# zyang1580/PDA

Hardware: AMD Instinct MI355X
Metric: users/sec full-catalogue top-K@50 (eval) (higher is better)
Workload: dtype f32; 1 GPU; C3: synthetic 1000000 users x 200000 items, d=128, PDA condition ((elu+1)*pop^0.22) head, masked top-K@50; ranks_seen=1

## Files before the change

### include/pda_hip_experimental.h

```cpp
#ifndef PDA_HIP_EXPERIMENTAL_H
#define PDA_HIP_EXPERIMENTAL_H

#include "pda_hip.h"

#ifdef __cplusplus
extern "C" {
#endif

int pda_score_topk_huge_splits(int n_users_blk, int n_items_local, int d);

int pda_topk_kth_value(const uint64_t* keys, int n_splits, int n_users_blk, int K, int pos, float* out, void* stream);
int pda_topk_remap_items(uint64_t* keys, size_t n_keys, const int32_t* gid, int n_gid, void* stream);
int pda_topk_seed_bounds(const uint64_t* keys, int n_splits, int n_users_blk, int K, int m, float* bounds, void* stream);
int pda_topk_seed_counts(const uint64_t* keys, int n_splits, int n_users_blk, int K, const float* bounds, int n_thr, int32_t* counts,
                         void* stream);
int pda_topk_seed_pick(const float* bounds, const int32_t* counts, int n_thr, int n_users_blk, int K, float* seed, void* stream);
int pda_topk_seed_refine(const uint64_t* keys, int n_splits, int n_users_blk, int K, float* lo, float* hi, float* mid, int32_t* counts,
                         int mode, void* stream);
int pda_score_topk4_phase_f32(const float* U, const float* I_shard, const void* prep, const float* pop_shard, const int32_t* users,
                              int n_users_blk, int item_offset, int n_items_local, int d, const int64_t* hist_indptr,
                              const int32_t* hist_indices, int hist_row_mode, int K, int head, int early_stop, int n_splits,
                              int phase, int warm_tiles, const float* seed, uint64_t* out_keys, void* workspace, void* stream);
int pda_score_topk4_phase_bf16(const uint16_t* U, const uint16_t* I_shard, const void* prep, const float* pop_shard,
                               const int32_t* users, int n_users_blk, int item_offset, int n_items_local, int d,
                               const int64_t* hist_indptr, const int32_t* hist_indices, int hist_row_mode, int K, int head,
                               int early_stop, int n_splits, int phase, int warm_tiles, const float* seed, uint64_t* out_keys,
                               void* workspace, void* stream);
int pda_score_topk4_phase_image_offsets(int n_users_blk, int n_items_local, int d, int n_splits, size_t* offs);
int pda_score_topk4_phase_user_image(const void* U, int bf16, const int32_t* users, int n_users_blk, int d, void* ufrag, float* unorm,
                                     void* stream);
int pda_score_topk4_phase_mask_table(const void* prep, int n_items_local, int d, int item_offset, const int64_t* hist_indptr,
                                     const int32_t* hist_indices, int n_rows, uint32_t* table, void* stream);
int pda_score_topk4_phase_masked_f32(const float* U, const float* I_shard, const void* prep, const float* pop_shard, const int32_t* users,
                                     int n_users_blk, int item_offset, int n_items_local, int d, const int64_t* hist_indptr,
                                     const int32_t* hist_indices, int hist_row_mode, int K, int head, int early_stop, int n_splits,
                                     const uint32_t* mask_table, int mask_table_rows, uint64_t* out_keys, void* workspace, void* stream);
int pda_score_topk4_phase_masked_bf16(const uint16_t* U, const uint16_t* I_shard, const void* prep, const float* pop_shard, const int32_t* users,
                                      int n_users_blk, int item_offset, int n_items_local, int d, const int64_t* hist_indptr,
                                      const int32_t* hist_indices, int hist_row_mode, int K, int head, int early_stop, int n_splits,
                                      const uint32_t* mask_table, int mask_table_rows, uint64_t* out_keys, void* workspace, void* stream);
int pda_score_topk4_phase_mask_rows(const void* prep, const int32_t* users, int n_users_blk, int item_offset, int n_items_local, int d,
                                    const int64_t* hist_indptr, const int32_t* hist_indices, int hist_row_mode, int warm_tiles, uint32_t* out,
                                    void* stream);
int pda_score_topk4_phase_mask_offsets(int n_users_blk, int n_items_local, int d, int n_splits, size_t* offs);

size_t pda_triplet_plan_bytes(int B);
size_t pda_triplet_plan_large_workspace_bytes(int B);
int pda_triplet_plan_large(const int32_t* users, const int32_t* pos, const int32_t* neg, int B, void* plan, void* workspace, void* stream);
size_t pda_bpr_step_plan_scratch_bytes(int B, int d);
int pda_triplet_plan(const int32_t* users, const int32_t* pos, const int32_t* neg, int B, int n_batches, void* plans, void* stream);
int pda_bpr_step_plan_f32(float* U, float* I, const int32_t* users, const int32_t* pos, const int32_t* neg, const float* pos_pop,
                          const float* neg_pop, int B, int d, float regs, float reg_div, float lr, const void* plan, float* scratch,
                          int exact, float* loss_acc, void* stream);
int pda_bpr_step_plan_bf16(uint16_t* U_bf16, uint16_t* I_bf16, float* U_master, float* I_master, const int32_t* users,
                           const int32_t* pos, const int32_t* neg, const float* pos_pop, const float* neg_pop, int B, int d,
                           float regs, float reg_div, float lr, const void* plan, float* scratch, float* loss_acc, void* stream);

int pda_sort_triplets_by_pos(int32_t* users, int32_t* pos, int32_t* neg, float* pos_pop, float* neg_pop, int B,
                             void* stream);

int pda_group_triplets_by_pos(int32_t* users, int32_t* pos, int32_t* neg, float* pos_pop, float* neg_pop, int B,
                              void* stream);

int pda_adam_mark_rows(const int32_t* users, const int32_t* pos, const int32_t* neg, int B, uint32_t* touched_u, uint32_t* touched_i, void* stream);
int pda_adam_dense_sweep3_f32(float* var_a, float* m_a, float* v_a, float* g_a, size_t rows_a, uint32_t* touched_a, float* var_b, float* m_b, float* v_b,
                              float* g_b, size_t rows_b, uint32_t* touched_b, int d, float lr_t, float beta1, float beta2, float eps, void* stream);

int pda_adam_rows_f32(float* var, float* m, float* v, float* g, const int32_t* rows, int n_rows, int d, float lr_t,
                      float beta1, float beta2, float eps, void* stream);

int pda_adam_lazy_f32(int phase, float* U, float* mU, float* vU, float* gU, int32_t* lastU, float* I, float* mI, float* vI,
                      float* gI, int32_t* lastI, const int32_t* users, const int32_t* pos, const int32_t* neg, int B, int d, int t,
                      const float* lr_tab, float beta1, float beta2, float eps, void* stream);
int pda_adam_lazy_sync_f32(float* var, float* m, float* v, int32_t* last, size_t n_rows, int d, int t, const float* lr_tab,
                           float beta1, float beta2, float eps, void* stream);
int pda_adam_lazy_dev_f32(int phase, float* U, float* mU, float* vU, float* gU, int32_t* lastU, float* I, float* mI, float* vI,
                          float* gI, int32_t* lastI, const int32_t* users, const int32_t* pos, const int32_t* neg, int B, int d,
// ... 41 lines not shown
```

### pda_amd/csrc/pda_score_topk_v4.hip

```cpp
#include "pda_v4_shared.h"
#include <cstdlib>
#include <type_traits>

using namespace pda_topk;

namespace {

constexpr int kCap4 = 57;
constexpr int kRing4 = 128;
constexpr int kWarmTiles = 4;
constexpr int kMainWaves = 8;
#ifndef PDA_W4_ABL
#define PDA_W4_ABL 0
#endif
#ifndef PDA_V4_ABL
#define PDA_V4_ABL 0
#endif
#ifdef PDA_V4_PROF
__device__ unsigned long long pda_prof4[24];
#define PROF_T0(v) const long long v = __builtin_readcyclecounter()
#define PROF_T1(v, slot) prof[slot] += (unsigned long long)(__builtin_readcyclecounter() - v)
#define PROF_INC(slot, x) prof[slot] += (unsigned long long)(x)
#define PROF_FLUSH(first, last) do { if (lane == 0) for (int pq = (first); pq <= (last); ++pq) atomicAdd(&pda_prof4[pq], prof[pq]); } while (0)
#else
// ... 17 lines not shown
    const float* sufA;
    const float* sufB;
    const int* pos_of;
    unsigned* stats;
    uint64_t* lists_ws;
    int32_t* regroup_ws;
    float* pred_ws;
    const int32_t* row_perm;
    const uint32_t* hmask_ws;
    const uint32_t* bloom;
    const int* prep_hdr;
    const float* seed;
    int n_users_blk, item_offset, n_items_local, hist_row_mode, K, n_splits, n_tiles;
    int warm_tiles;
    int warm_sorted;
    uint64_t* handover;
    const unsigned char* rows5;
    const float* meta5;
    const unsigned char* ufrag;
    const float* unorm;
    int prep_hdr_pop;
    int warm_final;
    int warm_shared;
    float* seed_out;
    const int* n_users_dev;
    int lists_empty;
    const float* tailA;
    const float* tailB;
    unsigned char* ufrag_out;
    float* unorm_out;
    float* kth_ws;
    const uint32_t* hmask_tab;
    int hmask_tab_rows;
};


template <int D, bool BF>
__global__ void __launch_bounds__(256) prep4_kernel(const void* __restrict__ I, const float* __restrict__ pop, const int* __restrict__ order,
                                                    int n, int n_pad, unsigned char* __restrict__ rows, int* __restrict__ pos_of,
                                                    int* __restrict__ hdr, unsigned char* __restrict__ rows5, int* __restrict__ meta5, u32x4* __restrict__ pinfo,
                                                    int f16img) {
    constexpr int TPR = D / 8, RB = row_bytes(D);
    const int pos = blockIdx.x * (256 / TPR) + threadIdx.x / TPR, e = threadIdx.x % TPR;
    if (pos >= n_pad) return;
    unsigned char* rp = rows + (size_t)pos * RB;
    float ss = 0.f, popv = 1.0f, rs = 0.f;
    int src = -1;
    if (pos < n) {
        src = pos;
        if (order) {
            src = order[pos];
            if (src < 0 || src >= n) { if (e == 0) atomicOr(hdr, 1); src = 0; }
            else if (e == 0 && atomicExch(&pos_of[src], pos) != -1) atomicOr(hdr, 1);
        } else if (e == 0) {
            pos_of[pos] = pos;
        }
        if (pop) popv = pop[src];
        const f32x4 a = pda_load4<BF>(I, (size_t)src * D + 8 * e);
        const f32x4 b = pda_load4<BF>(I, (size_t)src * D + 8 * e + 4);
        u32x4 hq, lq;
        split8(a, b, hq, lq);
        *reinterpret_cast<u32x4*>(rp + 16 * e) = hq;
#pragma unroll
        for (int k = 0; k < 4; ++k) ss += a[k] * a[k] + b[k] * b[k];
        {
            const float pv = pop ? ((popv == popv) ? popv : 0.f) : 1.0f;
// ... 571 lines not shown
        }
        if (g.kth_ws != nullptr) continue;
        if (g.handover != nullptr) {
            if (rb < g.n_users_blk && lane < CAP) g.handover[((size_t)split * g.n_users_blk + rb) * CAP + lane] = lane < c ? buf[lane] : 0ull;
            if (g.warm_final && rb < g.n_users_blk && lane < K) g.out_keys[((size_t)split * g.n_users_blk + rb) * K + lane] = lane < c ? buf[lane] : 0ull;
        } else if (rb < g.n_users_blk && lane < K) {
            const uint64_t k = lane < c ? buf[lane] : 0ull;
            g.out_keys[((size_t)split * g.n_users_blk + rb) * K + lane] = k;
        }
    }
    if (g.kth_ws != nullptr) {
        pda_wave_sync();
        const int rb0 = utile * kUserTile + wave * 32, nv = max(0, min(32, g.n_users_blk - rb0));
        if (lane < nv) {
            const uint64_t kl = my_lists[(size_t)lane * CAP + (K - 1)];
            g.kth_ws[(size_t)split * g.n_users_blk + rb0 + lane] = cntl[wave * 32 + lane] >= K ? pda_unordf((uint32_t)(kl >> 32)) : -INFINITY;
        }
        uint64_t* ob = g.out_keys + ((size_t)split * g.n_users_blk + rb0) * K;
        const int q64 = 64 / K, r64 = 64 % K;
        int rr = lane / K, p = lane % K;
        for (int i = lane; i < nv * K; i += 64) {
            ob[i] = p < cntl[wave * 32 + rr] ? my_lists[(size_t)rr * CAP + p] : 0ull;
            rr += q64;
            p += r64;
            if (p >= K) { p -= K; ++rr; }
        }
    }
    if (g.pred_ws != nullptr && lane < 32) {
        const int rb = utile * kUserTile + wave * 32 + lane;
        if (rb < g.n_users_blk) {
            g.pred_ws[2 * (size_t)rb] = predt[wave * 32 + lane];
            g.pred_ws[2 * (size_t)rb + 1] = nul[wave * 32 + lane];
        }
    }
}


#include "pda_v4_block_asm.h"
#ifndef PDA_V4_ASM
#define PDA_V4_ASM 1
#endif
#ifndef PDA_V4_RSLEEP
#define PDA_V4_RSLEEP 8
#endif
#ifndef PDA_V4_LSLEEP
#define PDA_V4_LSLEEP 1
#endif
#ifndef PDA_V4_GL
#define PDA_V4_GL 2
#endif
#ifndef PDA_V4_HANDOVER_WS
#define PDA_V4_HANDOVER_WS 1
#endif
#ifndef PDA_V4_ROWS_INTERLEAVED
#define PDA_V4_ROWS_INTERLEAVED 1
#endif
#ifndef PDA_V4_RESCORE_AHEAD
#define PDA_V4_RESCORE_AHEAD 1
#endif
#ifndef PDA_V4_RING_MANY
#define PDA_V4_RING_MANY 128
#endif
#ifndef PDA_V4_L256
#define PDA_V4_L256 3
#endif
#ifndef PDA_V4_ASM256
// ... 996 lines not shown
            int* bins = g.regroup_ws;
            int* bin_of = bins + 1024;
            int32_t* perm = bin_of + g.n_users_blk;
            if (hipMemsetAsync(bins, 0, 1024 * sizeof(int), stream) != hipSuccess) return PDA_ERR_LAUNCH;
            hipLaunchKernelGGL((stop_predict4_kernel<D, BF>), dim3((unsigned)((g.n_users_blk + 31) / 32)), dim3(256), 0, stream, g, bin_of);
            const unsigned hb = (unsigned)((g.n_users_blk + 4095) / 4096);
            hipLaunchKernelGGL(stop_hist4_kernel, dim3(hb), dim3(1024), 0, stream, bin_of, g.n_users_blk, bins);
            hipLaunchKernelGGL(stop_scan4_kernel, dim3(1), dim3(1024), 0, stream, bins);
            hipLaunchKernelGGL(stop_scatter4_kernel, dim3(hb), dim3(1024), 0, stream, bin_of, bins, g.n_users_blk, perm);
            PDA_CHECK_LAUNCH();
            gp.row_perm = perm;
            hipLaunchKernelGGL((sweep4_kernel<D, HEAD, BF, true, GM>), dim3((unsigned)(utiles * g.n_splits)), dim3(64 * G::WAVES), G::lds_total, stream, gp);
            PDA_CHECK_LAUNCH();
            return PDA_OK;
        }
        if (g.sufA != nullptr) {
            hipLaunchKernelGGL((sweep4_kernel<D, HEAD, BF, true, GM>), dim3((unsigned)(utiles * g.n_splits)), dim3(64 * G::WAVES), G::lds_total, stream, g);
            PDA_CHECK_LAUNCH();
            return PDA_OK;
        }
    } else if (g.sufA != nullptr) {
        return PDA_ERR_ARG;
    }
    hipLaunchKernelGGL((sweep4_kernel<D, HEAD, BF, false, GM>), dim3((unsigned)(utiles * g.n_splits)), dim3(64 * G::WAVES), G::lds_total, stream, g);
    PDA_CHECK_LAUNCH();
    return PDA_OK;
}

template <int D, int HEAD, bool BF>
int launch4_sweep(const Args4& g, hipStream_t stream, int geometry);

template <int D, int HEAD, bool BF>
int launch4(const Args4& g, int phase, hipStream_t stream, int geometry) {
    if (phase & 1) {
        constexpr int CAP = kCap4;
        const size_t smem = 32 * D * 4 + (size_t)kUserTile * (CAP * 8 + 8) + kUserTile * 2 * kWarmTiles * 4 + 256 + kUserTile * 8;
        static int attr_set = 0;
        if (!attr_set) {
            if (hipFuncSetAttribute(reinterpret_cast<const void*>(&warm4_kernel<D, HEAD, BF>), hipFuncAttributeMaxDynamicSharedMemorySize,
                                    (int)smem) != hipSuccess)
                return PDA_ERR_LAUNCH;
            attr_set = 1;
        }
        const int utiles = (g.n_users_blk + kUserTile - 1) / kUserTile;
        Args4 gw = g;
        if (g.warm_shared) {
            gw.n_splits = 1;
            gw.warm_shared = 0;
        }
        hipLaunchKernelGGL((warm4_kernel<D, HEAD, BF>), dim3((unsigned)(utiles * gw.n_splits)), dim3(kThreads), smem, stream, gw);
        PDA_CHECK_LAUNCH();
    }
    if ((g.n_tiles + g.n_splits - 1) / g.n_splits <= g.warm_tiles) return PDA_OK;
    if (phase & 2) {
        Args4 gs = g;
        if (g.warm_shared) gs.seed = g.seed_out;
        return launch4_sweep<D, HEAD, BF>(gs, stream, geometry);
    }
    return PDA_OK;
}

template <int D, int HEAD, bool BF>
int launch4_sweep(const Args4& g, hipStream_t stream, int geometry) {
    {
        if constexpr (HEAD == PDA_HEAD_POP) {
            if (geometry == 4 && g.sufA == nullptr && g.prep_hdr_pop != 0) return launch_sweep5<D, BF, true, D == 256 ? 128 : 256>(g, stream);
        }
        if constexpr (D <= 128) {
            if (geometry == 3) return launch_sweep4<D, HEAD, BF, 3>(g, stream);
        }
        return launch_sweep4<D, HEAD, BF, 0>(g, stream);
    }
    return PDA_OK;
}

int user_tile4(int d) { return d == 64 ? Geo4<64>::UT : d == 128 ? Geo4<128>::UT : Geo4<256>::UT; }
static bool lists_in_hbm4(int) { return true; }
struct Ws4 {
    size_t lists, bloom, hmask, regroup, handover, ufrag, unorm, seed, kth, total;
};
static Ws4 ws4_layout(int n_users_blk, int d, int n_splits) {
    auto al = [](size_t x) { return (x + 255) & ~(size_t)255; };
    Ws4 w{};
    w.lists = al(pda_score_topk_workspace_bytes(n_users_blk));
    size_t b = w.lists;
    if (lists_in_hbm4(d)) {
        const size_t ut = 1024;
        b += ((size_t)n_users_blk + ut - 1) / ut * (size_t)n_splits * ut * kCap4 * 8 + 256;
    }
    w.bloom = al(b);
    w.hmask = al(w.bloom + (size_t)n_users_blk * 128);
    w.regroup = al(w.hmask + ((size_t)n_users_blk + kUserTile - 1) / kUserTile * (size_t)n_splits * kUserTile * 2 * kWarmTiles * 4);
    w.handover = al(w.regroup + (1024 + 4 * (size_t)n_users_blk) * 4);
    w.total = w.handover + (size_t)n_splits * (size_t)n_users_blk * kCap4 * 8;
    w.ufrag = al(w.total);
    w.unorm = w.ufrag;
    {
        const size_t n_pad = ((size_t)n_users_blk + kUT5 - 1) / kUT5 * kUT5;
        w.unorm = w.ufrag + al(n_pad * 2 * (size_t)d);
        w.total = w.unorm + al(n_pad * 4);
    }
    w.seed = w.total;
    w.total = w.seed + al((size_t)n_users_blk * 4);
    w.kth = w.total;
    w.total = w.kth + al((size_t)n_splits * (size_t)n_users_blk * 4);
    return w;
}
extern "C" size_t pda_score_topk4_workspace_bytes(int n_users_blk, int n_items_local, int d, int n_splits) {
    if (n_users_blk <= 0 || n_items_local <= 0 || (d != 64 && d != 128 && d != 256)) return 0;
    if (n_splits <= 0) n_splits = pda_score_topk4_auto_splits(n_users_blk, n_items_local, d);
    return ws4_layout(n_users_blk, d, n_splits).total;
}

int run_score4(const void* U, const void* I_shard, bool bf16, const void* prep, const float* pop_shard, const int32_t* users,
               int n_users_blk, int item_offset, int n_items_local, int d, const int64_t* hist_indptr, const int32_t* hist_indices,
               int hist_row_mode, int K, int head, int early_stop, int n_splits, uint64_t* out_keys, void* workspace, hipStream_t s,
               int phase = 3, const float* seed = nullptr, int warm_tiles = 0, const int* n_users_dev = nullptr,
               const uint32_t* mask_table = nullptr, int mask_table_rows = 0) {
    if (!U || !I_shard || !prep || !users || !out_keys || !workspace) return PDA_ERR_ARG;
    if (n_users_blk <= 0 || n_items_local <= 0 || item_offset < 0) return PDA_ERR_ARG;
    if (K < 1 || K > PDA_MAX_K) return PDA_ERR_ARG;
    if (early_stop < 0 || (early_stop & ~0x7FF) != 0) return PDA_ERR_ARG;
    const bool warm_per_split = (early_stop & PDA_SWEEP_WARM_PER_SPLIT) != 0;
    int geometry = (early_stop & PDA_SWEEP_HUGE) ? 4 : (early_stop & PDA_SWEEP_MANY_CANDIDATES) ? 3 : 0;
    if (warm_tiles == 0) warm_tiles = (early_stop >> 4) & 7;
    early_stop &= 1;
    if (head != PDA_HEAD_RAW && head != PDA_HEAD_POP) return PDA_ERR_ARG;
    if (head == PDA_HEAD_POP && !pop_shard) return PDA_ERR_ARG;
    if (hist_indptr && !hist_indices) return PDA_ERR_ARG;
    if (d != 64 && d != 128 && d != 256) return PDA_ERR_UNSUPPORTED;
    if (K > kCap4 - 3) return PDA_ERR_UNSUPPORTED;
    if ((uint64_t)n_items_local > (1ull << 26)) return PDA_ERR_UNSUPPORTED;
    if (warm_tiles < 0 || warm_tiles > kWarmTiles) return PDA_ERR_ARG;
#ifndef PDA_V4_WARM_DEFAULT
#define PDA_V4_WARM_DEFAULT kWarmTiles
#endif
    if (warm_tiles == 0) warm_tiles = d <= 128 ? PDA_V4_WARM_DEFAULT : kWarmTiles;
    const bool from_empty = phase == 4;
    if (from_empty) {
        if (seed == nullptr) return PDA_ERR_ARG;
        phase = 2;
        warm_tiles = 0;
    } else if (phase < 1 || phase > 3) {
        return PDA_ERR_ARG;
    }
    if (n_splits <= 0) n_splits = pda_score_topk4_auto_splits(n_users_blk, n_items_local, d);
    const Prep4Layout L = prep4_layout(n_items_local, d);
    const unsigned char* pb = reinterpret_cast<const unsigned char*>(prep);
    if (((phase & 1) || from_empty) && hipMemsetAsync(workspace, 0, pda_score_topk_workspace_bytes(n_users_blk), s) != hipSuccess) return PDA_ERR_LAUNCH;
    const Ws4 W = ws4_layout(n_users_blk, d, n_splits);
    unsigned char* wsb = reinterpret_cast<unsigned char*>(workspace);
    const float* sA = reinterpret_cast<const float*>(pb + (head == PDA_HEAD_POP ? L.sufA : L.sufB));
    const float* sB = reinterpret_cast<const float*>(pb + (head == PDA_HEAD_POP ? L.sufB : L.sufR));
    Args4 g{U, I_shard, pop_shard, users, hist_indptr, hist_indices, out_keys, pb + L.rows,
            early_stop ? sA : nullptr, early_stop ? sB : nullptr, reinterpret_cast<const int*>(pb + L.pos_of),
            reinterpret_cast<unsigned*>(workspace), reinterpret_cast<uint64_t*>(wsb + W.lists), nullptr, nullptr, nullptr, nullptr, nullptr, reinterpret_cast<const int*>(pb + L.hdr), seed, n_users_blk, item_offset, n_items_local, hist_row_mode, K, n_splits, L.n_tiles, warm_tiles,
#ifdef PDA_V4_WARM_SORTED
            1, nullptr, pb + L.rows5, reinterpret_cast<const float*>(pb + L.meta5), nullptr, nullptr, 0};
#else
            (phase == 1 || (L.n_tiles + n_splits - 1) / n_splits <= warm_tiles) ? 1 : 0, nullptr,
            pb + L.rows5, reinterpret_cast<const float*>(pb + L.meta5), nullptr, nullptr, 0};
#endif
    if (phase == 3 && !g.warm_sorted && PDA_V4_HANDOVER_WS) g.handover = reinterpret_cast<uint64_t*>(wsb + W.handover);
    g.ufrag = wsb + W.ufrag;
    g.unorm = reinterpret_cast<const float*>(wsb + W.unorm);
    g.prep_hdr_pop = (head == PDA_HEAD_POP && pop_shard != nullptr) ? 1 : 0;
    g.warm_final = (geometry >= 4 && phase == 3 && g.handover != nullptr && g.prep_hdr_pop && !early_stop) ? 1 : 0;
    g.lists_empty = from_empty ? 1 : 0;
    g.n_users_dev = n_users_dev;
#ifndef PDA_V5_HANDOVER
    if (g.warm_final && geometry == 4) {
        g.handover = nullptr;
        g.kth_ws = reinterpret_cast<float*>(wsb + W.kth);
    }
#endif
#ifndef PDA_V5_UPREP
    if (geometry == 4 && phase == 3 && g.prep_hdr_pop && !early_stop && n_users_dev == nullptr && (L.n_tiles + n_splits - 1) / n_splits > warm_tiles) {
        g.ufrag_out = wsb + W.ufrag;
        g.unorm_out = reinterpret_cast<float*>(wsb + W.unorm);
    }
#endif
    if (g.prep_hdr_pop) {
        g.tailA = reinterpret_cast<const float*>(pb + L.sufA);
        g.tailB = reinterpret_cast<const float*>(pb + L.sufB);
    }
    if (phase == 3 && n_splits > 1 && seed == nullptr && !warm_per_split && L.n_tiles > n_splits * warm_tiles) {
        g.warm_shared = 1;
        g.seed_out = reinterpret_cast<float*>(wsb + W.seed);
    }
    if (hist_indptr && (phase & 2)) {
        uint32_t* bloom = reinterpret_cast<uint32_t*>(wsb + W.bloom);
        hipLaunchKernelGGL(hist_bloom4_kernel, dim3((unsigned)((n_users_blk + 31) / 32)), dim3(256), 0, s, users, hist_indptr, hist_indices,
                           hist_row_mode, n_users_blk, bloom, reinterpret_cast<const int*>(pb + L.hdr), head == PDA_HEAD_POP ? 1 : 0);
        PDA_CHECK_LAUNCH();
        g.bloom = bloom;
    }
    if (mask_table != nullptr && hist_indptr && hist_row_mode == PDA_HIST_BY_USER_ID && (phase & 1) && n_users_dev == nullptr &&
        (n_splits == 1 || g.warm_shared)) {
        g.hmask_tab = mask_table;
        g.hmask_tab_rows = mask_table_rows;
    } else if (hist_indptr && (phase & 1) && n_users_blk >= 98304) {
        uint32_t* hm = reinterpret_cast<uint32_t*>(wsb + W.hmask);
        const int utiles = (n_users_blk + kUserTile - 1) / kUserTile;
        Args4 gm = g;
        if (g.warm_shared) {
            gm.n_splits = 1;
            gm.warm_shared = 0;
        }
        hipLaunchKernelGGL(warm_mask4_kernel, dim3((unsigned)(utiles * gm.n_splits)), dim3(kThreads), 0, s, gm, hm);
        PDA_CHECK_LAUNCH();
        g.hmask_ws = hm;
    }
#ifndef PDA_V4_REGROUP_MIN
#define PDA_V4_REGROUP_MIN 98304
#endif
    if (early_stop && (phase & 2) && n_splits == 1 && n_users_blk >= PDA_V4_REGROUP_MIN) {
        g.regroup_ws = reinterpret_cast<int32_t*>(wsb + W.regroup);
        if (phase & 1) g.pred_ws = reinterpret_cast<float*>(g.regroup_ws + 1024 + 2 * (size_t)n_users_blk);
    }
    if (head == PDA_HEAD_RAW) {
        g.sufA = early_stop ? reinterpret_cast<const float*>(pb + L.sufA) : nullptr;
        g.sufB = early_stop ? reinterpret_cast<const float*>(pb + L.sufR) : nullptr;
    }
#define PDA_V4_(DD, BFV) (head == PDA_HEAD_POP ? launch4<DD, PDA_HEAD_POP, BFV>(g, phase, s, geometry) : launch4<DD, PDA_HEAD_RAW, BFV>(g, phase, s, geometry))
    switch (d) {
        case 64: return bf16 ? PDA_V4_(64, true) : PDA_V4_(64, false);
        case 128: return bf16 ? PDA_V4_(128, true) : PDA_V4_(128, false);
        case 256: return bf16 ? PDA_V4_(256, true) : PDA_V4_(256, false);
        default: return PDA_ERR_UNSUPPORTED;
    }
#undef PDA_V4_
}

__global__ void __launch_bounds__(256) kth_value_kernel(const uint64_t* __restrict__ keys, int S, int n_users, int K, int pos, float* __restrict__ out) {
// ... 332 lines not shown
```

### pda_amd/ops.py

```python
from __future__ import annotations

import math
import os
from typing import Optional, Tuple

import ctypes as C

import torch

from . import _lib
from ._lib import (HEAD_POP, HEAD_RAW, HIST_BY_BLOCK_ROW, HIST_BY_USER_ID, UPD_ANY_ORDER, UPD_DENSE_GRAD, UPD_NONE, UPD_USERS_DISTINCT,
                   UPD_SGD_FUSED, check, ptr, stream_ptr)

ADAM_BETA1, ADAM_BETA2, ADAM_EPS = 0.9, 0.999, 1e-8


def _need(t: Optional[torch.Tensor], dtype, name: str, optional=False):
    if t is None:
        if optional:
            return None
        raise ValueError(f"{name} is required")
    if not t.is_cuda:
        raise ValueError(f"{name} must live in HBM (cuda tensor); pda_amd has no CPU path")
    if t.dtype != dtype:
# ... 87 lines not shown

def item_prep_ordered(I_shard: torch.Tensor, pop_shard: Optional[torch.Tensor], order: Optional[torch.Tensor] = None):
    lib = _lib.load()
    if order is None:
        order = visiting_order(I_shard, pop_shard)
    n, d = I_shard.shape
    hit = _PREP_ORD_CACHE.get(id(I_shard))
    buf = None
    if hit is not None and hit[0]() is I_shard:
        buf = hit[5]
        same_pop = (hit[3] is None and pop_shard is None) or (hit[3] is not None and pop_shard is not None and hit[3]() is pop_shard
                                                             and hit[4] == pop_shard._version)
        if hit[1] == I_shard._version and hit[2] is order and same_pop:
            return buf, order
    bf = I_shard.dtype == torch.bfloat16
    if buf is None:
        nbytes = lib.pda_item_prep_ordered_bf16_bytes(n, d) if bf else lib.pda_item_prep_ordered_bytes(n, d)
        buf = torch.empty(nbytes, dtype=torch.uint8, device=I_shard.device)
    order = _need(order, torch.int32, "order")
    if order.numel() != n:
        raise ValueError("order must have one entry per local item row")
    fn = lib.pda_item_prep_ordered_bf16 if bf else lib.pda_item_prep_ordered_f32
    check(fn(ptr(I_shard), ptr(pop_shard), ptr(order), n, d, ptr(buf), stream_ptr()), "pda_item_prep_ordered")
    for k in [k for k, v in _PREP_ORD_CACHE.items() if v[0]() is None]:
        del _PREP_ORD_CACHE[k]
    _PREP_ORD_CACHE[id(I_shard)] = (weakref.ref(I_shard), I_shard._version, order,
                                    weakref.ref(pop_shard) if pop_shard is not None else None,
                                    pop_shard._version if pop_shard is not None else 0, buf)
    return buf, order


_PREP4_CACHE = {}
SWEEP_WARM_PER_SPLIT = 1024
TOPK_K_V4 = 54


def item_prep4(I_shard: torch.Tensor, pop_shard: Optional[torch.Tensor], order: Optional[torch.Tensor]) -> torch.Tensor:
    lib = _lib.load()
    n, d = I_shard.shape
    hit = _PREP4_CACHE.get(id(I_shard))
    buf = None
    if hit is not None and hit[0]() is I_shard:
        buf = hit[5]
        same_pop = (hit[3] is None and pop_shard is None) or (hit[3] is not None and pop_shard is not None and hit[3]() is pop_shard
                                                             and hit[4] == pop_shard._version)
        if hit[1] == I_shard._version and hit[2] is order and same_pop:
            return buf
    if buf is None:
        buf = torch.empty(lib.pda_item_prep4_bytes(n, d), dtype=torch.uint8, device=I_shard.device)
    if order is not None:
        order = _need(order, torch.int32, "order")
        if order.numel() != n:
            raise ValueError("order must have one entry per local item row")
    fn = lib.pda_item_prep4_bf16 if I_shard.dtype == torch.bfloat16 else lib.pda_item_prep4_f32
    check(fn(ptr(I_shard), ptr(pop_shard), ptr(order), n, d, ptr(buf), stream_ptr()), "pda_item_prep4")
    for k in [k for k, v in _PREP4_CACHE.items() if v[0]() is None]:
        del _PREP4_CACHE[k]
    _PREP4_CACHE[id(I_shard)] = (weakref.ref(I_shard), I_shard._version, order,
                                 weakref.ref(pop_shard) if pop_shard is not None else None,
                                 pop_shard._version if pop_shard is not None else 0, buf)
    return buf


_PREP7_CACHE = {}


# ... 339 lines not shown
        if cnt is not None:
            seed_sum(cnt)
        return seeded_finish(c)
    if n_splits_auto and out_given is None and impl == "v2" and funnel_applies(d, K, nu, nloc, head, prune, hist):
        return score_topk_funnel(U, I_shard, users, K, hist, item_offset, stats)
    if n_splits <= 0:
        n_splits = lib.pda_score_topk_auto_splits(nu, nloc)
    if out is None:
        out = torch.empty((n_splits, nu, K), dtype=torch.int64, device=U.device)
    elif out.shape != (n_splits, nu, K) or out.dtype != torch.int64:
        raise ValueError("out must be int64 [n_splits, Bu, K]")
    if impl == "v2" and score_kernel(d, K, nloc, prune, head) == "v4":
        order = visiting_order(I_shard, pop_shard if head == HEAD_POP else None) if prune else None
        prep = item_prep4(I_shard, pop_shard if head == HEAD_POP else None, order)
        forced_env = any(os.environ.get(k) for k in ("PDA_SCORE_LISTS", "PDA_SCORE_KERNEL", "PDA_HUGE_SPLITS"))
        plan = None
        if n_splits_auto and out_given is None and not forced_env and not (head == HEAD_POP and pop_shard is None):
            plan = score_plan(nu, nloc, d, K, head, prune, bf, hist)
            if plan["kernel"] != "v4":
                plan = None
        if plan is not None:
            n_splits = plan["n_splits"]
            out = torch.empty((n_splits, nu, K), dtype=torch.int64, device=U.device)
        elif n_splits_auto and out_given is None:
            n_splits = lib.pda_score_topk4_auto_splits(nu, nloc, d)
            if head == HEAD_POP and prune == "order" and d in (64, 128, 256) and not os.environ.get("PDA_SCORE_LISTS") and pop_shard is not None:
                n_splits = huge_splits(nu, nloc, d) or n_splits
            out = torch.empty((n_splits, nu, K), dtype=torch.int64, device=U.device)
        ws = torch.empty(lib.pda_score_topk4_workspace_bytes(nu, nloc, d, n_splits), dtype=torch.uint8, device=U.device)
        hint = plan["early_stop"] if plan is not None else ((1 if prune is True else 0) | few_candidates_hint(head, prune, nu, d, nloc, n_splits))
        es = hint | ((min(4, max(0, int(warm_tiles))) & 7) << 4)
        if os.environ.get("PDA_WARM_PER_SPLIT"):
            es |= SWEEP_WARM_PER_SPLIT
        tab = warm_mask_table(hist, prep, order, item_offset, nloc, d) if hist and (n_splits == 1 or not (es & SWEEP_WARM_PER_SPLIT)) else None
        if tab is not None:
            fn = lib.pda_score_topk4_phase_masked_bf16 if bf else lib.pda_score_topk4_phase_masked_f32
            check(fn(ptr(U), ptr(I_shard), ptr(prep), ptr(pop_shard), ptr(users), nu, item_offset, nloc, d,
                     ptr(hist.indptr), ptr(hist.indices), hist.mode, K, head, es, n_splits, ptr(tab), tab.shape[0],
                     ptr(out), ptr(ws), stream_ptr()), "pda_score_topk4_phase_masked")
        else:
            fn = lib.pda_score_topk4_bf16 if bf else lib.pda_score_topk4_f32
            check(fn(ptr(U), ptr(I_shard), ptr(prep), ptr(pop_shard), ptr(users), nu, item_offset, nloc, d,
                     ptr(hist.indptr) if hist else None, ptr(hist.indices) if hist else None, hist.mode if hist else 0,
                     K, head, es, n_splits, ptr(out), ptr(ws), stream_ptr()), "pda_score_topk4")
        if os.environ.get("PDA_CHECK_SWEEP_ERRORS"):
            err = int(ws[0:4].view(torch.int32)[0])
            if err != 0:
                raise RuntimeError("pda_score_topk4: the sweep reported protocol error %d" % err)
        if stats is not None:
            stats["tiles_scored"] = ws[8:16].view(torch.int64)
            stats["pairs_rescored"] = ws[4:8].view(torch.int32)
            stats["tiles_dense"] = ((nloc + 31) // 32) * ((nu + 127) // 128)
            stats["kernel_id"] = ws[16:20].view(torch.int32)
            stats["huge_entries"] = ws[20:24].view(torch.int32)
            stats["huge_free_halftiles"] = ws[28:32].view(torch.int32)
            stats["error"] = ws[0:4].view(torch.int32)
            stats["workspace"] = ws
            stats["n_splits"] = n_splits
            stats["warm_mask_table"] = tab
        return out
    if impl == "v2" and prune:
        prep, order = item_prep_ordered(I_shard, pop_shard if head == HEAD_POP else None)
        hist_ord = hist_reordered(hist, prep, order, item_offset, nloc, d) if hist else None
        ws = torch.empty(lib.pda_score_topk_workspace_bytes(nu), dtype=torch.uint8, device=U.device)
        fn = lib.pda_score_topk_ordered_bf16 if bf else lib.pda_score_topk_ordered_f32
        check(fn(ptr(U), ptr(I_shard), ptr(prep), ptr(pop_shard), ptr(users), nu, item_offset,
                                             nloc, d, ptr(hist.indptr) if hist else None,
                                             ptr(hist.indices) if hist else None, ptr(hist_ord), hist.mode if hist else 0,
                                             K, head, 0 if prune == "order" else 1, n_splits, ptr(out), ptr(ws), stream_ptr()),
              "pda_score_topk_ordered")
        if stats is not None:
            stats["tiles_scored"] = ws[8:16].view(torch.int64)
            stats["pairs_rescored"] = ws[4:8].view(torch.int32)
            stats["tiles_dense"] = ((nloc + 31) // 32) * ((nu + 127) // 128)
            stats["kernel_id"] = ws[16:20].view(torch.int32)
        return out
    if impl == "v2":
        prep = item_prep(I_shard)
        ws = torch.empty(lib.pda_score_topk_workspace_bytes(nu), dtype=torch.uint8, device=U.device)
        fn = lib.pda_score_topk_bf16 if bf else lib.pda_score_topk_prepped_f32
        check(fn(ptr(U), ptr(I_shard), ptr(prep), ptr(pop_shard), ptr(users), nu, item_offset,
                                             nloc, d, ptr(hist.indptr) if hist else None,
                                             ptr(hist.indices) if hist else None, hist.mode if hist else 0, K, head,
                                             n_splits, ptr(out), ptr(ws), stream_ptr()), "pda_score_topk_prepped_f32")
        return out
    check(lib.pda_score_topk_f32(ptr(U), ptr(I_shard), ptr(pop_shard), ptr(users), nu, item_offset, nloc, d,
                                 ptr(hist.indptr) if hist else None, ptr(hist.indices) if hist else None,
                                 hist.mode if hist else 0, K, head, n_splits, ptr(out), stream_ptr()),
# ... 1325 lines not shown
```

Baseline: 33.25 million users/s.

## Split warm phase into dense score kernel plus separate per-row select kernel

Replaces the single warm4 kernel, for the pop head with d<=128, with two kernels. The first scores the first warm tiles of items for every user into a workspace score matrix, using MFMA from an LDS-staged item block, and also writes the user bf16 fragments and norms. The second selects each row's top-K and K-th threshold by ballot-count binary search. It also skips the bloom kernel on the sweep5 path and makes the attribute caches per device. The aim is better occupancy and parallelism than the fused warm kernel, at the cost of an extra HBM round trip for the score matrix and a larger workspace.

```diff
diff --git a/include/pda_hip_experimental.h b/include/pda_hip_experimental.h
--- a/include/pda_hip_experimental.h
+++ b/include/pda_hip_experimental.h
@@ -43,6 +43,7 @@
                                     const int64_t* hist_indptr, const int32_t* hist_indices, int hist_row_mode, int warm_tiles, uint32_t* out,
                                     void* stream);
 int pda_score_topk4_phase_mask_offsets(int n_users_blk, int n_items_local, int d, int n_splits, size_t* offs);
+#define PDA_SWEEP_WARM_ONE_KERNEL 2048
 
 size_t pda_triplet_plan_bytes(int B);
 size_t pda_triplet_plan_large_workspace_bytes(int B);
diff --git a/pda_amd/csrc/pda_score_topk_v4.hip b/pda_amd/csrc/pda_score_topk_v4.hip
--- a/pda_amd/csrc/pda_score_topk_v4.hip
+++ b/pda_amd/csrc/pda_score_topk_v4.hip
@@ -73,6 +73,7 @@
     float* kth_ws;
     const uint32_t* hmask_tab;
     int hmask_tab_rows;
+    uint32_t* wscore;
 };
 
 
@@ -710,6 +711,325 @@
             g.pred_ws[2 * (size_t)rb] = predt[wave * 32 + lane];
             g.pred_ws[2 * (size_t)rb + 1] = nul[wave * 32 + lane];
         }
+    }
+}
+
+constexpr int kWS5Waves = 8, kWS5Threads = 64 * kWS5Waves;
+constexpr int kWarmPos = 64 * kWarmTiles;
+constexpr size_t warm_score5_lds(int d) { return (size_t)kWarmPos * d * 4 + kWarmPos * 8 + (size_t)kWS5Waves * 32 * 2 * kWarmTiles * 4; }
+
+template <int D, bool BF>
+__global__ void __launch_bounds__(kWS5Threads) warm_score5_kernel(Args4 g) {
+    extern __shared__ __attribute__((aligned(16))) unsigned char smem[];
+    constexpr int RB = row_bytes(D);
+    constexpr int NC = D / 8;
+    constexpr int CPR4 = D / 4;
+    float* Bt = reinterpret_cast<float*>(smem);
+    float* popw = Bt + kWarmPos * D;
+    int* idw = reinterpret_cast<int*>(popw + kWarmPos);
+    unsigned* hmask = reinterpret_cast<unsigned*>(idw + kWarmPos);
+
+    const int tid = threadIdx.x, lane = tid & 63, wave = tid >> 6;
+    const int j = lane & 31, h = lane >> 5;
+    const int nwarm = g.warm_tiles;
+    const int npos = 64 * nwarm;
+    for (int p = tid; p < npos; p += kWS5Threads) {
+        const float* tl = reinterpret_cast<const float*>(g.rows + (size_t)p * RB + 2 * D + 32);
+        popw[p] = tl[0];
+        idw[p] = reinterpret_cast<const int*>(tl)[1];
+    }
+    __syncthreads();
+    for (int id = tid; id < npos * CPR4; id += kWS5Threads) {
+        const int jj = id / CPR4, ch = id % CPR4;
+        *reinterpret_cast<f32x4*>(Bt + jj * D + 4 * (ch ^ swz<D>(jj & 31))) = pda_load4<BF>(g.I, (size_t)idw[jj] * D + 4 * ch);
+    }
+    if (blockIdx.x == 0) {
+        for (int p = tid; p < kWarmPos; p += kWS5Threads) g.wscore[p] = p < npos ? (uint32_t)idw[p] : 0u;
+        if (tid == 0) g.stats[8] = 5u;
+    }
+    __syncthreads();
+
+    uint32_t* scores = g.wscore + kWarmPos;
+    const int utiles_w = (g.n_users_blk + kUserTile - 1) / kUserTile;
+    const int nunits = utiles_w * (kUserTile / 32);
+    const int G = (int)gridDim.x, stride = G * kWS5Waves;
+    unsigned* hm_l = hmask + wave * 32 * 2 * kWarmTiles;
+    static_assert(2 * kWarmTiles == 8, "two 16-byte loads per row");
+
+    auto row_uid = [&](int unit) -> int {
+        const int rb = unit * 32 + j;
+        return (unit < nunits && rb < g.n_users_blk) ? g.users[rb] : 0;
+    };
+    auto load_rows = [&](int unit_x, int uid, f32x4 (&a)[NC], u32x4& hm, bool& hm_on) __attribute__((always_inline)) {
+        if (unit_x >= nunits) return;
+        const int rb = unit_x * 32 + j;
+#pragma unroll
+        for (int c = 0; c < NC; ++c) a[c] = pda_load4<BF>(g.U, (size_t)uid * D + 4 * h + 8 * c);
+        hm_on = false;
+        if (g.hmask_tab != nullptr) {
+            hm_on = rb < g.n_users_blk && (unsigned)uid < (unsigned)g.hmask_tab_rows;
+            hm = *reinterpret_cast<const u32x4*>(g.hmask_tab + (size_t)(hm_on ? uid : 0) * (2 * kWarmTiles) + 4 * h);
+        } else if (g.hmask_ws != nullptr) {
+            hm_on = true;
+            hm = *reinterpret_cast<const u32x4*>(g.hmask_ws + (size_t)rb * (2 * kWarmTiles) + 4 * h);
+        }
+    };
+    unsigned long long n_tiles_done = 0ull;
+    auto run_unit = [&](const int unit_in, f32x4 (&areg)[NC], const u32x4& hm_in, const bool hm_on) __attribute__((always_inline)) {
+        const int unit = __builtin_amdgcn_readfirstlane(unit_in);
+        const int row_blk = unit * 32 + j;
+        if (unit * 32 + 32 > g.n_users_blk) {
+            const f32x4 z = {0.f, 0.f, 0.f, 0.f};
+#pragma unroll
+            for (int c = 0; c < NC; ++c) areg[c] = row_blk < g.n_users_blk ? areg[c] : z;
+        }
+        const u32x4 hz = {0u, 0u, 0u, 0u};
+        const u32x4 hmv = hm_on ? hm_in : hz;
+        *reinterpret_cast<u32x4*>(hm_l + j * (2 * kWarmTiles) + 4 * h) = hmv;
+        {
+            constexpr int NK5 = D / 32;
+            unsigned char* fb = g.ufrag_out + ((size_t)(row_blk >> 4) * (NK5 * 64) + (size_t)(row_blk & 15)) * 16 + 8 * h;
+            float ssc[NC];
+#pragma unroll
+            for (int c = 0; c < NC; ++c) {
+                const f32x4 v = areg[c];
+                uint2 w;
+                w.x = bf16_rne(v[0]) | (bf16_rne(v[1]) << 16);
+                w.y = bf16_rne(v[2]) | (bf16_rne(v[3]) << 16);
+                *reinterpret_cast<uint2*>(fb + ((c >> 2) * 64 + 16 * (c & 3)) * 16) = w;
+                float ss = 0.f;
+#pragma unroll
+                for (int k = 0; k < 4; ++k) {
+                    const float sq = v[k] * v[k];
+                    ss += sq + __shfl_xor(sq, 32, 64);
+                }
+                ssc[c] = ss;
+                __builtin_amdgcn_sched_barrier(0);
+            }
+#pragma unroll
+            for (int o = NC / 2; o > 0; o >>= 1)
+#pragma unroll
+                for (int c = 0; c < o; ++c) ssc[c] += ssc[c + o];
+            if (h == 0) g.unorm_out[row_blk] = sqrtf(ssc[0]) * 1.0009765625f * 1.0001f;
+        }
+        if ((unit & (kUserTile / 32 - 1)) == 0) n_tiles_done += (unsigned long long)(2 * nwarm);
+        pda_wave_sync();
+        const int j_lane = j, h_lane = h;
+#pragma unroll 1
+        for (int ht = 0; ht < 2 * nwarm; ++ht) {
+            int j = j_lane, h = h_lane;
+#if defined(__HIP_DEVICE_COMPILE__)
+            asm volatile("" : "+v"(j), "+v"(h));
+#endif
+            const int bswz = swz<D>(j);
+            const float* brow = Bt + (ht * 32 + j) * D;
+            f32x16 acc0 = zero16v(), acc1 = zero16v();
+            f32x4 b0 = *reinterpret_cast<const f32x4*>(brow + 4 * (h ^ bswz));
+            f32x4 b1 = *reinterpret_cast<const f32x4*>(brow + 4 * ((2 + h) ^ bswz));
+#pragma unroll
+            for (int c = 0; c < NC; c += 2) {
+                f32x4 n0 = b0, n1 = b1;
+                if (c + 2 < NC) {
+                    n0 = *reinterpret_cast<const f32x4*>(brow + 4 * ((2 * c + 4 + h) ^ bswz));
+                    n1 = *reinterpret_cast<const f32x4*>(brow + 4 * ((2 * c + 6 + h) ^ bswz));
+                }
+#pragma unroll
+                for (int q = 0; q < 4; ++q) {
+                    acc0 = __builtin_amdgcn_mfma_f32_32x32x2f32(areg[c][q], b0[q], acc0, 0, 0, 0);
+                    acc1 = __builtin_amdgcn_mfma_f32_32x32x2f32(areg[c + 1][q], b1[q], acc1, 0, 0, 0);
+                }
+                __builtin_amdgcn_sched_barrier(0);
+                b0 = n0;
+                b1 = n1;
+            }
+            const f32x16 accx = acc0 + acc1;
+            const bool okw = (ht * 32 + j) < g.n_items_local;
+            const float pv = popw[ht * 32 + j];
+            const unsigned hb_mine = hm_l[j * (2 * kWarmTiles) + ht];
+            const bool any_hb = __any(hb_mine != 0u);
+            const uint32_t soff = (uint32_t)(unit * 32 + 4 * h) * (uint32_t)npos + (uint32_t)(ht * 32 + j);
+#pragma unroll
+            for (int r = 0; r < 16; ++r) {
+                const int row = (r & 3) + 8 * (r >> 2) + 4 * h;
+                float sc = accx[r];
+                sc = (sc > 0.0f ? sc + 1.0f : __expf(sc)) * pv;
+                bool p = okw && (sc >= -INFINITY);
+                if (any_hb) {
+                    const uint32_t hbr = (uint32_t)__shfl((int)hb_mine, row, 64);
+                    if ((hbr >> j) & 1u) p = false;
+                }
+                scores[soff + (uint32_t)((r & 3) + 8 * (r >> 2)) * (uint32_t)npos] = p ? pda_ordf(sc + 0.0f) : 0u;
+            }
+        }
+        pda_wave_sync();
+    };
+    int unit = (int)blockIdx.x + G * wave;
+    f32x4 ra[NC], rb_[NC];
+    u32x4 ha = {0u, 0u, 0u, 0u}, hb = {0u, 0u, 0u, 0u};
+    bool oa = false, ob = false;
+    load_rows(unit, row_uid(unit), ra, ha, oa);
+    int uid_n = row_uid(unit + stride);
+    while (unit < nunits) {
+        load_rows(unit + stride, uid_n, rb_, hb, ob);
+        uid_n = row_uid(unit + 2 * stride);
+        run_unit(unit, ra, ha, oa);
+        unit += stride;
+        if (unit >= nunits) break;
+        load_rows(unit + stride, uid_n, ra, ha, oa);
+        uid_n = row_uid(unit + 2 * stride);
+        run_unit(unit, rb_, hb, ob);
+        unit += stride;
+    }
+    if (lane == 0 && n_tiles_done != 0ull) atomicAdd(reinterpret_cast<unsigned long long*>(g.stats + 2), n_tiles_done);
+    if ((int)blockIdx.x == (nunits - 1) % G) {
+        const size_t r0 = (size_t)utiles_w * kUserTile, r1 = ((size_t)g.n_users_blk + kUT5 - 1) / kUT5 * kUT5;
+        const u32x4 z = {0u, 0u, 0u, 0u};
+        for (size_t q = r0 * (2 * D) + (size_t)tid * 16; q < r1 * (2 * D); q += (size_t)kWS5Threads * 16) *reinterpret_cast<u32x4*>(g.ufrag_out + q) = z;
+        for (size_t r = r0 + tid; r < r1; r += kWS5Threads) g.unorm_out[r] = 0.f;
+    }
+}
+
+constexpr int kSelRows = 16;
+__global__ void __launch_bounds__(256) __attribute__((amdgpu_waves_per_eu(8))) warm_select5_kernel(Args4 g) {
+    constexpr int CAP = kCap4;
+    __shared__ uint64_t lists[4][2][64];
+    const int tid = threadIdx.x, lane = tid & 63, wave = tid >> 6;
+    const int K = g.K, n = g.n_users_blk;
+    const int npos = 64 * g.warm_tiles;
+    const uint32_t* scores = g.wscore + kWarmPos;
+    const int rb0 = ((int)blockIdx.x * 4 + wave) * kSelRows;
+    if (rb0 >= n) return;
+    const u32x4 idv = *reinterpret_cast<const u32x4*>(g.wscore + 4 * lane);
+    uint32_t klo[4];
+#pragma unroll
+    for (int q = 0; q < 4; ++q) klo[q] = 0xFFFFFFFFu - (uint32_t)(g.item_offset + (int)idv[q]);
+    const bool lane_on = 4 * lane < npos;
+    float kth_mine = -INFINITY;
+
+    auto count32 = [&](const u32x4& v, uint32_t t) __attribute__((always_inline)) -> int {
+        return __popcll(__ballot(v[0] >= t)) + __popcll(__ballot(v[1] >= t)) + __popcll(__ballot(v[2] >= t)) + __popcll(__ballot(v[3] >= t));
+    };
+    auto key_of = [&](const u32x4& v, int q) __attribute__((always_inline)) -> uint64_t { return ((uint64_t)v[q] << 32) | (uint64_t)klo[q]; };
+    auto count64 = [&](const u32x4& v, uint64_t t) __attribute__((always_inline)) -> int {
+        int c = 0;
+#pragma unroll
+        for (int q = 0; q < 4; ++q) c += __popcll(__ballot(key_of(v, q) >= t));
+        return c;
+    };
+
+#pragma unroll 1
+    for (int it = 0; it < kSelRows; it += 2) {
+        if (rb0 + it >= n) break;
+        u32x4 v[2];
+        uint32_t t[2], hi[2];
+        int ct[2];
+        bool need[2];
+#pragma unroll
+        for (int s = 0; s < 2; ++s) {
+            const int rb = rb0 + it + s;
+            const u32x4 z = {0u, 0u, 0u, 0u};
+            v[s] = (lane_on && rb < n) ? *reinterpret_cast<const u32x4*>(scores + (size_t)rb * npos + 4 * lane) : z;
+        }
+#pragma unroll
+        for (int s = 0; s < 2; ++s) {
+            ct[s] = count32(v[s], 1u);
+            t[s] = 1u;
+            hi[s] = 0u;
+            need[s] = ct[s] > CAP;
+        }
+        if (need[0] || need[1]) {
+#pragma unroll
+            for (int s = 0; s < 2; ++s) {
+                uint32_t mx = max(max(v[s][0], v[s][1]), max(v[s][2], v[s][3])), mn = 0xFFFFFFFFu;
+#pragma unroll
+                for (int q = 0; q < 4; ++q) mn = min(mn, v[s][q] != 0u ? v[s][q] : 0xFFFFFFFFu);
+#pragma unroll
+                for (int o = 32; o >= 1; o >>= 1) {
+                    mx = max(mx, (uint32_t)__shfl_xor((int)mx, o, 64));
+                    mn = min(mn, (uint32_t)__shfl_xor((int)mn, o, 64));
+                }
+                hi[s] = (uint32_t)__builtin_amdgcn_readfirstlane((int)mx) + 1u;
+                if (need[s]) t[s] = (uint32_t)__builtin_amdgcn_readfirstlane((int)mn);
+            }
+            for (int step = 0; step < 40; ++step) {
+                const bool open0 = need[0] && ct[0] > CAP && hi[0] - t[0] > 1u;
+                const bool open1 = need[1] && ct[1] > CAP && hi[1] - t[1] > 1u;
+                if (!(open0 || open1)) break;
+                const uint32_t mid0 = open0 ? t[0] + ((hi[0] - t[0]) >> 1) : t[0];
+                const uint32_t mid1 = open1 ? t[1] + ((hi[1] - t[1]) >> 1) : t[1];
+                const int c0 = count32(v[0], mid0), c1 = count32(v[1], mid1);
+                if (open0) {
+                    if (c0 >= K) { t[0] = mid0; ct[0] = c0; } else { hi[0] = mid0; }
+                }
+                if (open1) {
+                    if (c1 >= K) { t[1] = mid1; ct[1] = c1; } else { hi[1] = mid1; }
+                }
+            }
+        }
+        uint64_t thr[2];
+#pragma unroll
+        for (int s = 0; s < 2; ++s) {
+            thr[s] = (uint64_t)t[s] << 32;
+            if (ct[s] > CAP) {
+                uint64_t lo64 = thr[s], hi64 = (uint64_t)(t[s] + 1u) << 32;
+                for (int step = 0; step < 40 && ct[s] > CAP && hi64 - lo64 > 1ull; ++step) {
+                    const uint64_t mid = lo64 + ((hi64 - lo64) >> 1);
+                    const int c = count64(v[s], mid);
+                    if (c >= K) { lo64 = mid; ct[s] = c; } else { hi64 = mid; }
+                }
+                thr[s] = lo64;
+            }
+        }
+        int cs[2];
+#pragma unroll
+        for (int s = 0; s < 2; ++s) {
+            uint64_t* buf = lists[wave][s];
+            int run = 0;
+#pragma unroll
+            for (int q = 0; q < 4; ++q) {
+                const uint64_t key = key_of(v[s], q);
+                const bool p = key >= thr[s];
+                const uint64_t bm = __ballot(p);
+                const int slot = run + (int)__builtin_amdgcn_mbcnt_hi((uint32_t)(bm >> 32), __builtin_amdgcn_mbcnt_lo((uint32_t)bm, 0));
+                if (p && slot < 64) buf[slot] = key;
+                run += __popcll(bm);
+            }
+            cs[s] = min(run, CAP);
+            if (lane >= cs[s]) buf[lane] = 0ull;
+        }
+        pda_wave_sync();
+        uint64_t key[2];
+        int rank[2] = {0, 0};
+        key[0] = lists[wave][0][lane];
+        key[1] = lists[wave][1][lane];
+        const int cm = max(cs[0], cs[1]);
+        for (int jj = 0; jj < cm; jj += 4) {
+#pragma unroll
+            for (int s = 0; s < 2; ++s) {
+                const uint64_t* buf = lists[wave][s];
+                const uint64_t k0 = buf[jj], k1 = buf[jj + 1], k2 = buf[jj + 2], k3 = buf[jj + 3];
+                rank[s] += ((k0 > key[s]) ? 1 : 0) + ((k1 > key[s]) ? 1 : 0) + ((k2 > key[s]) ? 1 : 0) + ((k3 > key[s]) ? 1 : 0);
+            }
+        }
+        pda_wave_sync();
+#pragma unroll
+        for (int s = 0; s < 2; ++s)
+            if (lane < cs[s]) lists[wave][s][rank[s]] = key[s];
+        pda_wave_sync();
+#pragma unroll
+        for (int s = 0; s < 2; ++s) {
+            const int rb = rb0 + it + s;
+            if (rb < n) {
+                if (lane < K) g.out_keys[(size_t)rb * K + lane] = lists[wave][s][lane];
+                const uint64_t kl = lists[wave][s][K - 1];
+                if (lane == it + s) kth_mine = cs[s] >= K ? pda_unordf((uint32_t)(kl >> 32)) : -INFINITY;
+            }
+        }
+        pda_wave_sync();
+    }
+    if (lane < kSelRows && rb0 + lane < n) {
+        g.kth_ws[rb0 + lane] = kth_mine;
+        if (g.seed_out != nullptr) g.seed_out[rb0 + lane] = kth_mine;
     }
 }
 
@@ -1772,15 +2092,43 @@
 
 template <int D, int HEAD, bool BF>
 int launch4(const Args4& g, int phase, hipStream_t stream, int geometry) {
-    if (phase & 1) {
+    bool warm_two = false;
+    if constexpr (HEAD == PDA_HEAD_POP && D <= 128) warm_two = (phase & 1) && g.wscore != nullptr;
+    if constexpr (HEAD == PDA_HEAD_POP && D <= 128) {
+        if (warm_two) {
+            constexpr size_t smem = warm_score5_lds(D);
+            constexpr int kMaxDev = 64;
+            static int cu_of_dev[kMaxDev] = {};
+            int dev = 0;
+            if (hipGetDevice(&dev) != hipSuccess || dev < 0 || dev >= kMaxDev) return PDA_ERR_LAUNCH;
+            if (cu_of_dev[dev] == 0) {
+                int cus = 0;
+                if (hipDeviceGetAttribute(&cus, hipDeviceAttributeMultiprocessorCount, dev) != hipSuccess || cus <= 0) return PDA_ERR_LAUNCH;
+                if (hipFuncSetAttribute(reinterpret_cast<const void*>(&warm_score5_kernel<D, BF>), hipFuncAttributeMaxDynamicSharedMemorySize,
+                                        (int)smem) != hipSuccess)
+                    return PDA_ERR_LAUNCH;
+                cu_of_dev[dev] = cus;
+            }
+            const int n_cu = cu_of_dev[dev];
+            const int nunits = (g.n_users_blk + kUserTile - 1) / kUserTile * (kUserTile / 32);
+            hipLaunchKernelGGL((warm_score5_kernel<D, BF>), dim3((unsigned)(n_cu < nunits ? n_cu : nunits)), dim3(kWS5Threads), smem, stream, g);
+            PDA_CHECK_LAUNCH();
+            hipLaunchKernelGGL(warm_select5_kernel, dim3((unsigned)((g.n_users_blk + 4 * kSelRows - 1) / (4 * kSelRows))), dim3(256), 0, stream, g);
+            PDA_CHECK_LAUNCH();
+        }
+    }
+    if ((phase & 1) && !warm_two) {
         constexpr int CAP = kCap4;
         const size_t smem = 32 * D * 4 + (size_t)kUserTile * (CAP * 8 + 8) + kUserTile * 2 * kWarmTiles * 4 + 256 + kUserTile * 8;
-        static int attr_set = 0;
-        if (!attr_set) {
+        constexpr int kMaxDev = 64;
+        static char attr_set[kMaxDev] = {};
+        int dev = 0;
+        if (hipGetDevice(&dev) != hipSuccess || dev < 0 || dev >= kMaxDev) return PDA_ERR_LAUNCH;
+        if (!attr_set[dev]) {
             if (hipFuncSetAttribute(reinterpret_cast<const void*>(&warm4_kernel<D, HEAD, BF>), hipFuncAttributeMaxDynamicSharedMemorySize,
                                     (int)smem) != hipSuccess)
                 return PDA_ERR_LAUNCH;
-            attr_set = 1;
+            attr_set[dev] = 1;
         }
         const int utiles = (g.n_users_blk + kUserTile - 1) / kUserTile;
         Args4 gw = g;
@@ -1817,7 +2165,7 @@
 int user_tile4(int d) { return d == 64 ? Geo4<64>::UT : d == 128 ? Geo4<128>::UT : Geo4<256>::UT; }
 static bool lists_in_hbm4(int) { return true; }
 struct Ws4 {
-    size_t lists, bloom, hmask, regroup, handover, ufrag, unorm, seed, kth, total;
+    size_t lists, bloom, hmask, regroup, handover, ufrag, unorm, seed, kth, wscore, total;
 };
 static Ws4 ws4_layout(int n_users_blk, int d, int n_splits) {
     auto al = [](size_t x) { return (x + 255) & ~(size_t)255; };
@@ -1844,6 +2192,8 @@
     w.total = w.seed + al((size_t)n_users_blk * 4);
     w.kth = w.total;
     w.total = w.kth + al((size_t)n_splits * (size_t)n_users_blk * 4);
+    w.wscore = w.total;
+    w.total = w.wscore + al((size_t)kWarmPos * 4 + ((size_t)n_users_blk + kUserTile - 1) / kUserTile * kUserTile * kWarmPos * 4);
     return w;
 }
 extern "C" size_t pda_score_topk4_workspace_bytes(int n_users_blk, int n_items_local, int d, int n_splits) {
@@ -1860,8 +2210,9 @@
     if (!U || !I_shard || !prep || !users || !out_keys || !workspace) return PDA_ERR_ARG;
     if (n_users_blk <= 0 || n_items_local <= 0 || item_offset < 0) return PDA_ERR_ARG;
     if (K < 1 || K > PDA_MAX_K) return PDA_ERR_ARG;
-    if (early_stop < 0 || (early_stop & ~0x7FF) != 0) return PDA_ERR_ARG;
+    if (early_stop < 0 || (early_stop & ~0xFFF) != 0) return PDA_ERR_ARG;
     const bool warm_per_split = (early_stop & PDA_SWEEP_WARM_PER_SPLIT) != 0;
+    const bool warm_one_kernel = (early_stop & PDA_SWEEP_WARM_ONE_KERNEL) != 0;
     int geometry = (early_stop & PDA_SWEEP_HUGE) ? 4 : (early_stop & PDA_SWEEP_MANY_CANDIDATES) ? 3 : 0;
     if (warm_tiles == 0) warm_tiles = (early_stop >> 4) & 7;
     early_stop &= 1;
@@ -1928,7 +2279,11 @@
         g.warm_shared = 1;
         g.seed_out = reinterpret_cast<float*>(wsb + W.seed);
     }
-    if (hist_indptr && (phase & 2)) {
+    const bool warm_two = g.ufrag_out != nullptr && g.kth_ws != nullptr && d <= 128 && !warm_one_kernel && (n_splits == 1 || g.warm_shared) &&
+                          n_users_blk <= (1 << 21);
+    if (warm_two) g.wscore = reinterpret_cast<uint32_t*>(wsb + W.wscore);
+    const bool sweep5 = head == PDA_HEAD_POP && geometry == 4 && !early_stop && g.prep_hdr_pop != 0;
+    if (hist_indptr && (phase & 2) && !sweep5) {
         uint32_t* bloom = reinterpret_cast<uint32_t*>(wsb + W.bloom);
         hipLaunchKernelGGL(hist_bloom4_kernel, dim3((unsigned)((n_users_blk + 31) / 32)), dim3(256), 0, s, users, hist_indptr, hist_indices,
                            hist_row_mode, n_users_blk, bloom, reinterpret_cast<const int*>(pb + L.hdr), head == PDA_HEAD_POP ? 1 : 0);
@@ -1939,7 +2294,7 @@
         (n_splits == 1 || g.warm_shared)) {
         g.hmask_tab = mask_table;
         g.hmask_tab_rows = mask_table_rows;
-    } else if (hist_indptr && (phase & 1) && n_users_blk >= 98304) {
+    } else if (hist_indptr && (phase & 1) && (n_users_blk >= 98304 || warm_two)) {
         uint32_t* hm = reinterpret_cast<uint32_t*>(wsb + W.hmask);
         const int utiles = (n_users_blk + kUserTile - 1) / kUserTile;
         Args4 gm = g;
diff --git a/pda_amd/ops.py b/pda_amd/ops.py
--- a/pda_amd/ops.py
+++ b/pda_amd/ops.py
@@ -143,6 +143,7 @@
 
 _PREP4_CACHE = {}
 SWEEP_WARM_PER_SPLIT = 1024
+SWEEP_WARM_ONE_KERNEL = 2048
 TOPK_K_V4 = 54
 
 
@@ -548,6 +549,8 @@
         es = hint | ((min(4, max(0, int(warm_tiles))) & 7) << 4)
         if os.environ.get("PDA_WARM_PER_SPLIT"):
             es |= SWEEP_WARM_PER_SPLIT
+        if os.environ.get("PDA_WARM_ONE_KERNEL"):
+            es |= SWEEP_WARM_ONE_KERNEL
         tab = warm_mask_table(hist, prep, order, item_offset, nloc, d) if hist and (n_splits == 1 or not (es & SWEEP_WARM_PER_SPLIT)) else None
         if tab is not None:
             fn = lib.pda_score_topk4_phase_masked_bf16 if bf else lib.pda_score_topk4_phase_masked_f32
@@ -570,6 +573,7 @@
             stats["kernel_id"] = ws[16:20].view(torch.int32)
             stats["huge_entries"] = ws[20:24].view(torch.int32)
             stats["huge_free_halftiles"] = ws[28:32].view(torch.int32)
+            stats["warm_kernels"] = ws[32:36].view(torch.int32)
             stats["error"] = ws[0:4].view(torch.int32)
             stats["workspace"] = ws
             stats["n_splits"] = n_splits
```

Result: faster. 34.29 million users/s, median of 6 (+3.1%).
